# yardenas/ethz-safe-learning

Hardware: AMD Instinct MI355X
Metric: planning steps/sec (CEM-MPC, N=2000 K=5 H=30) (higher is better)
Workload: dtype f32

## Files before the change

ethz_safe_learning_amd/_capi.py:

```python
from __future__ import annotations

import ctypes as C
import os

CEM_ABI_VERSION = 4
CEM_MAX_ACT = 32
CEM_MAX_COST_KINDS = 4
CEM_COMM_ID_BYTES = 128
CEM_MAX_BATCH = 256
CEM_TRAIN_MAX_BATCH = 4096
CEM_INIT_COLD, CEM_INIT_EXPLICIT, CEM_INIT_SHIFT = 0, 1, 2
CEM_VARIANT_CEM, CEM_VARIANT_SAFE, CEM_VARIANT_COST = 0, 1, 2
CEM_PARTICLES_MEAN, CEM_PARTICLES_LOWER_TAIL = 0, 1
CEM_CONSTRAINT_BETA, CEM_CONSTRAINT_BUDGET = 0, 1
CEM_REFIT_UNIFORM, CEM_REFIT_SOFTMAX = 0, 1
CEM_NOISE_WHITE, CEM_NOISE_MIXED = 0, 1
CEM_FORWARD_SPLIT, CEM_FORWARD_ALL = 0, 1

_HERE = os.path.dirname(os.path.abspath(__file__))
LIB_PATH = os.environ.get('CEM_MPC_LIB') or os.path.join(_HERE, 'lib', 'libcem_mpc_gfx950.so')

EXPORTED_SYMBOLS = [
    'cem_abi_version', 'cem_status_string', 'cem_last_hip_error', 'cem_weight_blob_floats',
    'cem_packed_weight_floats', 'cem_workspace_bytes', 'cem_pack_weights_host', 'cem_plan_tiles_host', 'cem_plan_segments_host', 'cem_rollout_residency',
    'cem_planner_create', 'cem_planner_destroy', 'cem_planner_layout', 'cem_planner_set_weights', 'cem_planner_set_weights_dev',
    'cem_planner_set_normaliser', 'cem_planner_plan', 'cem_plan_begin', 'cem_plan_rollout', 'cem_plan_select',
    'cem_plan_end', 'cem_comm_unique_id', 'cem_planner_comm_init', 'cem_planner_comm_destroy', 'cem_planner_comm_ranks', 'cem_plan_exchange', 'cem_planner_graph_status', 'cem_planner_launches_per_iteration', 'cem_planner_rollout_path', 'cem_unfold_sequences', 'cem_compute_objective', 'cem_scorer_reward', 'cem_scorer_cost', 'cem_fill_noise', 'cem_philox_words', 'cem_planner_set_timing', 'cem_planner_last_timing', 'cem_planner_last_timing_detail', 'cem_planner_select_mode', 'cem_planner_inject_fault',
    'cem_batch_workspace_bytes', 'cem_batch_planner_create', 'cem_planner_plan_batch', 'cem_planner_batch_capacity',
    'cem_planner_set_warm_start', 'cem_planner_set_initial_distribution', 'cem_planner_set_init_mode', 'cem_planner_reset_carry',
    'cem_planner_get_carry', 'cem_planner_set_carry_slots', 'cem_planner_set_particle_objective', 'cem_planner_get_particle_objective',
    'cem_planner_set_constraint', 'cem_planner_get_constraint', 'cem_planner_set_cost_budget', 'cem_planner_constraint_costs',
    'cem_planner_set_refit', 'cem_planner_get_refit', 'cem_planner_refit_stats',
    'cem_planner_set_action_noise', 'cem_planner_get_action_noise', 'cem_planner_action_noise_dev',
    'cem_trainer_workspace_bytes', 'cem_trainer_blob_floats', 'cem_trainer_create', 'cem_trainer_destroy', 'cem_trainer_set_state',
    'cem_trainer_get_state', 'cem_trainer_weights_dev', 'cem_trainer_step', 'cem_trainer_steps', 'cem_trainer_eval', 'cem_trainer_forward',
]


class CemScorer(C.Structure):
    _fields_ = [
        ('goal_mode', C.c_int32), ('goal_lo', C.c_int32), ('goal_hi', C.c_int32),
        ('lidar_max_dist', C.c_float), ('goal_size', C.c_float), ('goal_reached_dist', C.c_float), ('reward_distance', C.c_float),
        ('reward_goal', C.c_float), ('reward_clip', C.c_float),
        ('constrain_indicator', C.c_int32), ('n_cost_kinds', C.c_int32),
        ('cost_lo', C.c_int32 * CEM_MAX_COST_KINDS), ('cost_hi', C.c_int32 * CEM_MAX_COST_KINDS),
        ('cost_size', C.c_float * CEM_MAX_COST_KINDS),
    ]


class CemConfig(C.Structure):
    _fields_ = [
        ('abi_version', C.c_int32), ('obs_dim', C.c_int32), ('act_dim', C.c_int32),
        ('units', C.c_int32), ('n_layers', C.c_int32), ('activation', C.c_int32), ('ensemble_size', C.c_int32),
        ('particles', C.c_int32), ('n_samples', C.c_int32), ('horizon', C.c_int32),
        ('n_elite', C.c_int32), ('iterations', C.c_int32),
        ('smoothing', C.c_float), ('one_minus_smoothing', C.c_float), ('stddev_threshold', C.c_float), ('noise_stddev', C.c_float),
        ('variant', C.c_int32), ('posterior_mean_threashold', C.c_float),
        ('sampling_propagation', C.c_int32), ('scale_features', C.c_int32),
        ('act_lb', C.c_float * CEM_MAX_ACT), ('act_ub', C.c_float * CEM_MAX_ACT),
        ('act_mu0', C.c_float * CEM_MAX_ACT), ('act_sigma0', C.c_float * CEM_MAX_ACT),
# ... 43 lines not shown
    vp, fp, i32p = C.c_void_p, C.POINTER(C.c_float), C.POINTER(C.c_int32)
    cfgp = C.POINTER(CemConfig)
    lib.cem_abi_version.restype = C.c_int
    lib.cem_status_string.restype = C.c_char_p
    lib.cem_status_string.argtypes = [C.c_int]
    lib.cem_last_hip_error.restype = C.c_int
    for f in ('cem_weight_blob_floats', 'cem_packed_weight_floats', 'cem_workspace_bytes'):
        getattr(lib, f).restype = C.c_size_t
        getattr(lib, f).argtypes = [cfgp]
    lib.cem_pack_weights_host.argtypes = [cfgp, vp, vp]
    lib.cem_plan_tiles_host.argtypes = [cfgp, i32p, i32p, vp, C.c_int32]
    lib.cem_plan_segments_host.argtypes = [cfgp, i32p, i32p]
    lib.cem_rollout_residency.argtypes = [C.c_int32, C.c_int32, i32p, i32p]
    lib.cem_planner_create.argtypes = [cfgp, vp, C.c_size_t, vp, C.POINTER(vp)]
    lib.cem_planner_destroy.argtypes = [vp]
    lib.cem_planner_layout.argtypes = [vp, C.POINTER(CemLayout)]
    lib.cem_planner_set_weights.argtypes = [vp, vp, C.c_size_t]
    lib.cem_planner_set_weights_dev.argtypes = [vp, vp, C.c_size_t]
    lib.cem_planner_set_normaliser.argtypes = [vp, vp, vp]
    lib.cem_planner_plan.argtypes = [vp, vp, C.c_uint64, C.c_uint64, vp, vp, vp, vp, fp, i32p]
    lib.cem_plan_begin.argtypes = [vp, vp, C.c_uint64, C.c_uint64, vp, vp]
    lib.cem_plan_rollout.argtypes = [vp, C.c_int32]
    lib.cem_plan_select.argtypes = [vp, C.c_int32]
    lib.cem_plan_end.argtypes = [vp, vp, vp, fp, i32p]
    lib.cem_unfold_sequences.argtypes = [vp, vp, vp, C.c_int32, C.c_int32, vp, C.c_uint64, C.c_uint64, vp, vp, vp]
    lib.cem_comm_unique_id.argtypes = [vp]
    lib.cem_planner_comm_init.argtypes = [vp, vp, C.c_int32, C.c_int32]
    lib.cem_planner_comm_destroy.argtypes = [vp]
    lib.cem_plan_exchange.argtypes = [vp]
    lib.cem_planner_graph_status.argtypes = [vp, i32p]
    lib.cem_planner_comm_ranks.argtypes = [vp, i32p]
    lib.cem_planner_launches_per_iteration.argtypes = [vp, i32p]
    lib.cem_planner_rollout_path.argtypes = [vp, i32p]
    lib.cem_compute_objective.argtypes = [vp, vp, C.c_int32, C.c_int32, vp]
    lib.cem_scorer_reward.argtypes = [vp, vp, vp, C.c_int32, vp, vp]
    lib.cem_scorer_cost.argtypes = [vp, vp, C.c_int32, vp]
    lib.cem_fill_noise.argtypes = [vp, C.c_uint64, C.c_uint64, vp, vp, vp]
    lib.cem_philox_words.argtypes = [vp, C.c_uint64, C.c_uint64] + [C.c_uint32] * 6 + [vp]
    lib.cem_planner_select_mode.argtypes = [vp, i32p]
    lib.cem_planner_inject_fault.argtypes = [vp, C.c_int32]
    lib.cem_planner_set_timing.argtypes = [vp, C.c_int32]
    lib.cem_planner_last_timing.argtypes = [vp, fp, i32p, fp]
    lib.cem_planner_last_timing_detail.argtypes = [vp, fp, fp]
    lib.cem_batch_workspace_bytes.restype = C.c_size_t
    lib.cem_batch_workspace_bytes.argtypes = [cfgp, C.c_int32]
    lib.cem_batch_planner_create.argtypes = [cfgp, C.c_int32, vp, C.c_size_t, vp, C.POINTER(vp)]
    lib.cem_planner_plan_batch.argtypes = [vp, C.c_int32, vp, C.c_uint64, vp, vp, vp, vp, vp, vp, vp]
    lib.cem_planner_batch_capacity.argtypes = [vp, i32p]
    lib.cem_planner_set_warm_start.argtypes = [vp, C.POINTER(CemWarmStart)]
    lib.cem_planner_set_initial_distribution.argtypes = [vp, C.c_int32, vp, vp]
    lib.cem_planner_set_init_mode.argtypes = [vp, C.c_int32, C.c_int32]
    lib.cem_planner_reset_carry.argtypes = [vp, C.c_int32]
    lib.cem_planner_get_carry.argtypes = [vp, C.c_int32, vp, vp, i32p]
    lib.cem_planner_set_carry_slots.argtypes = [vp, C.c_int32, vp]
    lib.cem_planner_set_particle_objective.argtypes = [vp, C.c_int32, C.c_int32]
    lib.cem_planner_get_particle_objective.argtypes = [vp, i32p, i32p]
    lib.cem_planner_set_constraint.argtypes = [vp, C.c_int32, C.c_int32]
    lib.cem_planner_get_constraint.argtypes = [vp, i32p, i32p]
    lib.cem_planner_set_cost_budget.argtypes = [vp, vp, C.c_int32]
    lib.cem_planner_constraint_costs.argtypes = [vp, C.c_int32, vp, C.c_int32]
    lib.cem_planner_set_refit.argtypes = [vp, C.c_int32, C.c_float]
    lib.cem_planner_get_refit.argtypes = [vp, i32p, fp]
    lib.cem_planner_refit_stats.argtypes = [vp, C.c_int32, vp, C.c_int32]
    lib.cem_planner_set_action_noise.argtypes = [vp, C.c_int32, vp]
    lib.cem_planner_get_action_noise.argtypes = [vp, i32p, vp]
    lib.cem_planner_action_noise_dev.argtypes = [vp, C.POINTER(vp), C.POINTER(C.c_size_t)]
# ... 28 lines not shown
```

ethz_safe_learning_amd/csrc/cem_capi.hip:

```cpp
#include "cem_device.h"
#include "cem_rollout_lean.h"
#include "cem_score.h"
#include "cem_refit_weighted.h"
#include "cem_noise_mix.h"
#include "cem_train.h"
#include "cem_train_tile.h"
#include "cem_forward.h"
#include "cem_rollout_split.h"
#include "cem_rollout_wide.h"
#include "cem_pack.h"
#include "../../include/cem_mpc.h"

#include <dlfcn.h>
#include <link.h>

#include <algorithm>
#include <atomic>
#include <chrono>
#include <cmath>
#include <cstdio>
#include <cstdlib>
#include <cstring>
#include <limits>
#include <mutex>
// ... 1968 lines not shown
    int n = 0;
    NCCLCHK(r->CommCount(h->comm, &n));
    *n_ranks_out = n;
    return CEM_OK;
}

int cem_planner_comm_destroy(cem_planner_t *h)
{
    if (!h) return CEM_ERR_INVALID_ARG;
    if (h->in_plan) return CEM_ERR_STATE;
    if (h->comm) {
        HIPCHK(hipStreamSynchronize(h->stream));
        if (Rccl *r = rccl()) r->CommDestroy(h->comm);
        h->comm = nullptr;
        drop_graph(h);
    }
    return CEM_OK;
}

int cem_planner_graph_status(const cem_planner_t *h, int32_t *status_out)
{
    if (!h || !status_out) return CEM_ERR_INVALID_ARG;
    *status_out = h->graph_ready ? 1 : (h->graph_failed ? 2 : 0);
    return CEM_OK;
}

int cem_planner_rollout_path(const cem_planner_t *h, int32_t *path_out)
{
    if (!h || !path_out) return CEM_ERR_INVALID_ARG;
    *path_out = (h->lean_rollout && h->noise_kind != CEM_NOISE_MIXED) ? 1 : 0;
    return CEM_OK;
}

int cem_planner_launches_per_iteration(const cem_planner_t *h, int32_t *launches_out)
{
    if (!h || !launches_out) return CEM_ERR_INVALID_ARG;
    const int mode = select_mode_now(h);
    *launches_out = 1 + (h->sample_in_rollout ? 0 : 1) + (folds_reduce(h) ? 0 : 1) + (mode == 2 ? 8 : (mode == 3 ? 2 : 1)) +
                    (h->refit_kind == CEM_REFIT_SOFTMAX ? 1 : 0);
    return CEM_OK;
}

int cem_plan_exchange(cem_planner_t *h)
{
    if (!h) return CEM_ERR_INVALID_ARG;
    if (!h->in_plan || !h->comm) return CEM_ERR_STATE;
    return enqueue_exchange(h);
}

static int ensure_scratch(cem_planner *h, size_t bytes)
{
    if (bytes <= h->scratch_bytes) return CEM_OK;
    if (h->scratch) { HIPCHK(hipStreamSynchronize(h->stream)); HIPCHK(hipFree(h->scratch)); h->scratch = nullptr; h->scratch_bytes = 0; }
    const size_t want = align256(bytes + bytes / 2);
    HIPCHK(hipMalloc((void **)&h->scratch, want));
    h->scratch_bytes = want;
    return CEM_OK;
}

static int upload_key(cem_planner *h, uint64_t seed, uint64_t call)
{
    CtrlBlock *c = h->h_ctrl;
    c->seed_lo = (uint32_t)seed; c->seed_hi = (uint32_t)(seed >> 32); c->call_lo = (uint32_t)call; c->call_hi = (uint32_t)(call >> 32);
    HIPCHK(hipMemcpyAsync(h->ws + h->lay.ctrl, c, 16, hipMemcpyHostToDevice, h->stream));
    return CEM_OK;
}
// ... 449 lines not shown
```

ethz_safe_learning_amd/csrc/cem_rollout_lean.h:

```cpp
#pragma once
#include "cem_device.h"

#define CEM_LEAN_ACT_LDS_BYTES(H_, AZ_) (((size_t)(H_) + 1) * (AZ_) * (32 + 17 * 16))
#define CEM_LEAN_LDS_BYTES(H_, AZ_) (CEM_ROLLOUT_LDS_BYTES(1) + CEM_LEAN_ACT_LDS_BYTES(H_, AZ_))
#define CEM_LEAN_ACT_LDS_MAX 16384

__attribute__((weak)) hipError_t launch_rollout_lean(const RolloutParams &p, int grid, hipStream_t st, bool seg);
```

ethz_safe_learning_amd/csrc/cem_rollout_lean.hip:

```cpp
#define CEM_DEVICE_PRIMITIVES_ONLY
#include "cem_rollout_lean.h"

namespace {

template <int V> struct LeanConst { static constexpr int value = V; };

template <int KF, int NOWN, bool L0IN>
__device__ __forceinline__ void cem_lean_stage(f4 (&acc0)[1], f4 (&acc1)[1], f4 (&hB)[CEM_NG][1], WRing &wq, const char *const *rb, const int xoff)
{
    static_assert(KF % 4 == 0, "stage lengths must keep the ring phase");
#pragma unroll
    for (int P = 0; P < KF; ++P) {
        wq.slot[(P + 3) & 3] = wq.ld(wq.pos);
        wq.pos = (wq.pos + 1 == wq.n) ? 0 : wq.pos + 1;
        __builtin_amdgcn_sched_barrier(0);
        if (P == 1) {
            __syncthreads();
#pragma unroll
            for (int Q = NOWN; Q < KF; ++Q) hB[Q][0] = *reinterpret_cast<const f4 *>(rb[Q - NOWN] + xoff + (Q - NOWN) * 1024);
        }
        const AGroup g = wq.slot[P & 3];
        const int Pb = (!L0IN && P < 2) ? (P ^ 1) : P;
#pragma unroll
        for (int r = 0; r < 4; ++r) {
            acc0[0] = CEM_MFMA(g.a[r], hB[P][0][r], acc0[0]);
            acc1[0] = CEM_MFMA(g.b[r], hB[Pb][0][r], acc1[0]);
        }
    }
}

template <bool SEG>
__device__ __forceinline__ void cem_lean_tile(const RolloutParams &p, char *smem, const int tile_idx, const int t_begin, const int t_end)
{
    constexpr int RC = 1, NFW = 1;
    const int tid = (int)((threadIdx.x + 64u * (unsigned)((tile_idx + (tile_idx >> 8)) & 3)) & 255u);
    const int w = __builtin_amdgcn_readfirstlane(tid >> 6);
    const int lane = tid & 63;
    const int j = lane & 15, q = lane >> 4;
    const TileDesc td = p.tiles[tile_idx];
    const bool resumed = SEG && t_begin > 0;
    const int wbk = 0;
    const __amdgpu_buffer_rsrc_t seg_rs = __builtin_amdgcn_make_buffer_rsrc(
        SEG ? const_cast<f4 *>(p.seg_state + (size_t)(tile_idx - p.n_pinned) * (2 * 256 + 64)) : const_cast<f4 *>(p.wpack), 0, (2 * 256 + 64) * 16, 0x00020000);
    const int O = p.O, A = p.A, H = p.H, AZ = (A + 3) >> 2;
    constexpr int XB = CEM_NG * 1024;
    float *part = reinterpret_cast<float *>(smem + 2 * XB);
    const CtrlBlock *const ctrl = p.ctrl;
    const PhiloxKey key = cem_key(ctrl);
    const float rscale = p.sampling ? CEM_BM_RSCALE : 0.0f;

    const int member_u = __builtin_amdgcn_readfirstlane(td.member);
    WRing wq;
    wq.init(p.wpack + (size_t)member_u * p.member_stride_f4 + p.wave_off_f4[w], lane, (int)p.wave_groups[w]);

    const __amdgpu_buffer_rsrc_t et_rs = __builtin_amdgcn_make_buffer_rsrc(
        const_cast<float *>(p.etab + (size_t)member_u * (CEM_ET_ROWS + p.L) * CEM_U), 0, (CEM_ET_ROWS + p.L) * CEM_U * 4, 0x00020000);
    const int tab_v = 64 * w + 16 * q;
    const int bias_v = 128 * w + 16 * q;
    const char *tabl = smem + 2 * XB + CEM_PART_FLOATS * 4;
    const char *actl = tabl + CEM_TAB_LDS_BYTES;
    {
        const int ht = (int)threadIdx.x;
        *reinterpret_cast<f4 *>(const_cast<char *>(tabl) + ht * 16) = cem_ld_tab(et_rs, (ht & 31) * 16, (ht >> 5) * 512);
        const int HA = H * A;
// ... 21 lines not shown
                float v = 0.f;
                if (f < O) v = td.s0_base < 0 ? ctrl->state[f] : p.s0[(size_t)(td.s0_base + slot0) * O + f];
                s[0][0][r] = v;
            }
        }
    }

    const int zq = 4 * w + q - (O >> 2);
    const bool actlane = zq >= 0 && zq < AZ;
    const bool wact = 4 * w + 3 >= (O >> 2) && 4 * w < (O >> 2) + AZ;
    const int zc = actlane ? zq : 0;
    const uint32_t pc0 = (uint32_t)((actlane ? td.act_base : td.noise_row_base) + slot0);
    const uint32_t pc2 = actlane ? ((uint32_t)zc | (CEM_STREAM_ACT << 16)) : ((uint32_t)(4 * w + q) | (CEM_STREAM_MODEL << 16));
    const uint32_t pc1 = ((uint32_t)p.it << 16) + (actlane ? 1u : 0u);
    const float prs = actlane ? CEM_BM_RSCALE : rscale;
    const char *const actl_v = actl + zc * 32;
#define CEM_LEAN_ACTION(DST, E_, T_) do { \
        const char *m_ = actl_v + (T_) * AZ * 32, *b_ = actl_v + H * AZ * 32; \
        const f4 sg_ = *reinterpret_cast<const f4 *>(m_), mu_ = *reinterpret_cast<const f4 *>(m_ + 16); \
        const f4 lb_ = *reinterpret_cast<const f4 *>(b_), ub_ = *reinterpret_cast<const f4 *>(b_ + 16); \
        f4 v_ = (E_) * sg_; v_ = v_ + mu_; \
        _Pragma("unroll") for (int r = 0; r < 4; ++r) DST[r] = fminf(fmaxf(v_[r], lb_[r]), ub_[r]); } while (0)
    const bool act_keep = actlane && j < td.cnt && td.row_base < p.Nloc;
    char *const stage = const_cast<char *>(actl) + (H + 1) * AZ * 32;
    char *const stage_v = stage + ((act_keep ? j : 16) * (H + 1) * AZ + zc) * 16;
#define CEM_LEAN_KEEP(V_, T_) do { *reinterpret_cast<f4 *>(stage_v + (T_) * AZ * 16) = (V_); } while (0)

    float d_prev = 0.f, c_prev = 0.f, cum = 0.f;
    bool done = false;
    const int nk = 1 + p.sc.n_cost;
    const float csz[4] = {p.sc.cost_size[0], p.sc.cost_size[1], p.sc.cost_size[2], p.sc.cost_size[3]};
    const float ind_cap = p.sc.indicator ? 1.0f : __builtin_inff(), clipv = p.sc.reward_clip > 0.f ? p.sc.reward_clip : __builtin_inff();
    const __amdgpu_buffer_rsrc_t cost_rs = __builtin_amdgcn_make_buffer_rsrc(p.costs, 0, p.costs ? (uint32_t)(H * p.Bloc) : 0u, 0x00020000);

    f4 hB[CEM_NG][RC];
    if (resumed) {
        const f4 x = cem_ld_coherent(seg_rs, (256 + tid) * 16);
        hB[0][0] = x;
        *reinterpret_cast<f4 *>(smem + (w * 64 + lane) * 16) = x;
        if (w == wbk) {
            const f4 b = cem_ld_coherent(seg_rs, (2 * 256 + lane) * 16);
            d_prev = b[0]; c_prev = b[1]; cum = b[2]; done = b[3] != 0.f;
        }
    } else {
        float pm[2][RC];
        pm[0][0] = __builtin_inff(); pm[1][0] = __builtin_inff();
        const int tv = tab_v;
        const f4 mn4 = CEM_TAB(tabl, CEM_ET_NMIN, tv), rd4 = CEM_TAB(tabl, CEM_ET_RDELTA, tv);
        const f4 isact4 = CEM_TAB(tabl, CEM_ET_ACT, tv);
        const f4 sel0 = CEM_TAB(tabl, CEM_ET_SEL0, tv), sel1 = CEM_TAB(tabl, CEM_ET_SEL1, tv);
        const f4 e0 = cem_normal4(pc0, 0u, (uint32_t)p.it, (uint32_t)zc, CEM_STREAM_ACT, key);
        const f4 sn = s[0][0];
        f4 xin = sn;
        if (wact) {
            f4 act4; CEM_LEAN_ACTION(act4, e0, 0);
            CEM_LEAN_KEEP(act4, 0);
            xin = __builtin_elementwise_fma(isact4, act4, sn);
        }
        cem_scorer_terms(sn, p.sc.D, sel0, sel1, pm[0][0], pm[1][0]);
        const f4 x = cem_sub4(xin, mn4) * rd4;
        *reinterpret_cast<f4 *>(smem + (w * 64 + lane) * 16) = x;
        hB[0][0] = x;
        CEM_RARE_KINDS_AND_STORE(RC, NFW, p, part, w, q, j, nk, s, pm, tab_v, CEM_SEL0_LDS, tabl);
    }
    f4 nb0 = cem_ld_tab(et_rs, bias_v, CEM_ET_ROWS * 512);
    f4 nb1 = cem_ld_tab(et_rs, bias_v + 64, CEM_ET_ROWS * 512);

    const char *rbh[6], *rb0[3];
#pragma unroll
    for (int k = 0; k < 6; ++k) rbh[k] = smem + lane * 16 + (k < 2 * w ? 0 : 2048);
#pragma unroll
    for (int k = 0; k < 3; ++k) rb0[k] = smem + lane * 16 + (k < w ? 0 : 1024);
    char *const pubh = smem + (2 * w * 64 + lane) * 16, *const pub0 = smem + (w * 64 + lane) * 16;
    const bool prio_rot = !(SEG && tile_idx >= p.n_pinned);
    const int prio_r0 = (tile_idx >> 8) % 3;
    auto step = [&](auto XW0, const int t, const bool first) __attribute__((always_inline)) {
        int xw = decltype(XW0)::value;
        if (prio_rot) {
            const int lvl = (t + prio_r0) % 3;
            if (lvl == 0) __builtin_amdgcn_s_setprio(0); else if (lvl == 1) __builtin_amdgcn_s_setprio(1); else __builtin_amdgcn_s_setprio(2);
        }
#define CEM_RELU_PUBLISH() do { \
            f4 h0 = acc0[0], h1 = acc1[0]; \
            _Pragma("unroll") for (int r = 0; r < 4; ++r) { h0[r] = fmaxf(h0[r], 0.f); h1[r] = fmaxf(h1[r], 0.f); } \
            *reinterpret_cast<f4 *>(pubh + xw) = h0; \
            *reinterpret_cast<f4 *>(pubh + xw + 1024) = h1; \
            hB[0][0] = h0; hB[1][0] = h1; \
            xw ^= XB; } while (0)
#define CEM_NEXT_BIAS(LN) do { \
            nb0 = cem_ld_tab(et_rs, bias_v, (CEM_ET_ROWS + (LN)) * 512); \
            nb1 = cem_ld_tab(et_rs, bias_v + 64, (CEM_ET_ROWS + (LN)) * 512); } while (0)
        {
            f4 acc0[RC], acc1[RC];
            acc0[0] = nb0; acc1[0] = nb1;
            CEM_NEXT_BIAS(1);
            cem_lean_stage<4, 1, true>(acc0, acc1, hB, wq, rb0, xw ^ XB);
            if (!(resumed && first)) CEM_BOOKKEEP(p, td, part, w, wbk, lane, nk, csz, ind_cap, clipv, cost_rs, d_prev, c_prev, cum, done, t - 1);
            CEM_RELU_PUBLISH();
        }
#pragma unroll
        for (int l = 1; l < 4; ++l) {
            f4 acc0[RC], acc1[RC];
            acc0[0] = nb0; acc1[0] = nb1;
            CEM_NEXT_BIAS(l + 1 < 4 ? l + 1 : 0);
            cem_lean_stage<CEM_NG, 2, false>(acc0, acc1, hB, wq, rbh, xw ^ XB);
            CEM_RELU_PUBLISH();
        }
#undef CEM_RELU_PUBLISH
#undef CEM_NEXT_BIAS

        float pm[2][RC];
        pm[0][0] = __builtin_inff(); pm[1][0] = __builtin_inff();
        const int tn = (t + 1 < H) ? t + 1 : H - 1;
        {
            const int Fo = w;
            const int tv = tab_v;
            f4 accm[RC], accv[RC];
            accm[0] = CEM_TAB(tabl, CEM_ET_BMU, tv); accv[0] = CEM_TAB(tabl, CEM_ET_BVAR, tv);
            if (Fo < p.KB_obs) cem_lean_stage<CEM_NG, 2, false>(accm, accv, hB, wq, rbh, xw ^ XB);
            else __syncthreads();
            const f4 e4 = cem_normal4(pc0, pc1 + (uint32_t)t, 0u, pc2, 0u, key, prs);
            const f4 mn4 = CEM_TAB(tabl, CEM_ET_NMIN, tv), rd4 = CEM_TAB(tabl, CEM_ET_RDELTA, tv);
            const f4 om4 = CEM_TAB(tabl, CEM_ET_OBS, tv), isact4 = CEM_TAB(tabl, CEM_ET_ACT, tv);
            const f4 sel0 = CEM_TAB(tabl, CEM_ET_SEL0, tv), sel1 = CEM_TAB(tabl, CEM_ET_SEL1, tv);

            const f4 mu = accm[0];
            const f4 var = cem_softplus4(accv[0]) + 1e-4f;
            f4 sd;
#pragma unroll
            for (int r = 0; r < 4; ++r) sd[r] = __builtin_amdgcn_sqrtf(var[r]);
            const f4 d = mu + sd * e4;
            const f4 sn = s[0][0] + d * om4;
            s[0][0] = sn;
            cem_scorer_terms(sn, p.sc.D, sel0, sel1, pm[0][0], pm[1][0]);
            f4 xin = sn;
            if (wact) {
                f4 act4; CEM_LEAN_ACTION(act4, e4, tn);
                CEM_LEAN_KEEP(act4, t + 1);
                xin = __builtin_elementwise_fma(isact4, act4, sn);
            }
            const f4 x = cem_sub4(xin, mn4) * rd4;
            *reinterpret_cast<f4 *>(pub0 + xw) = x;
            hB[0][0] = x;
        }
        CEM_RARE_KINDS_AND_STORE(RC, NFW, p, part, w, q, j, nk, s, pm, tab_v, CEM_SEL0_LDS, tabl);
    };
    for (int t = t_begin; t < t_end; t += 2) {
        step(LeanConst<XB>{}, t, t == t_begin);
        if (t + 1 >= t_end) break;
        step(LeanConst<0>{}, t + 1, false);
    }
#undef CEM_LEAN_ACTION
#undef CEM_LEAN_KEEP
    __syncthreads();
    CEM_BOOKKEEP(p, td, part, w, wbk, lane, nk, csz, ind_cap, clipv, cost_rs, d_prev, c_prev, cum, done, t_end - 1);
    if (td.row_base < p.Nloc) {
        const int tlo = resumed ? t_begin + 1 : 0, thi = t_end < H ? t_end : H - 1;
        const int per = (thi - tlo + 1) * A;
        const float *const stagef = reinterpret_cast<const float *>(stage);
        for (int idx = (int)threadIdx.x; idx < td.cnt * per; idx += 256) {
            const int row = idx / per, rem = idx - row * per, tt = tlo + rem / A, a = rem - (rem / A) * A;
            p.actions_w[((size_t)(td.act_base + row) * H + tt) * A + a] = stagef[((row * (H + 1) + tt) * AZ) * 4 + a];
        }
    }
    if (!SEG || t_end == H) {
        if (w == wbk && lane < td.cnt) p.ret[td.row_base + lane] = cum;
    } else {
        cem_st_coherent(seg_rs, tid * 16, s[0][0]);
        cem_st_coherent(seg_rs, (256 + tid) * 16, hB[0][0]);
        if (w == wbk) cem_st_coherent(seg_rs, (2 * 256 + lane) * 16, (f4){d_prev, c_prev, cum, done ? 1.0f : 0.0f});
    }
}

}

__global__ __launch_bounds__(256) void cem_rollout_lean_kernel(const RolloutParams p)
{
    extern __shared__ __attribute__((aligned(16))) char smem[];
    if (p.check_done && p.ctrl->done) return;
    cem_lean_tile<false>(p, smem, (int)blockIdx.x, 0, p.H);
}

__global__ __launch_bounds__(256) void cem_rollout_lean_seg_kernel(const RolloutParams p)
{
    extern __shared__ __attribute__((aligned(16))) char smem[];
    __shared__ uint32_t item_s;
    if (p.check_done && p.ctrl->done) return;
    if ((int)blockIdx.x < p.n_pinned) {
        cem_lean_tile<true>(p, smem, (int)blockIdx.x, 0, p.H);
        return;
    }
    __builtin_amdgcn_s_setprio(CEM_FLOAT_PRIO);
    const uint32_t n_float = (uint32_t)(p.n_tiles - p.n_pinned);
    if (threadIdx.x == 0) {
        const uint32_t ticket = atomicAdd(p.seg_queue, 1u);
        uint32_t item = (((uint32_t)p.n_pinned + ticket) << 8);
        if (ticket >= n_float) {
            const uint32_t *slot = p.seg_flags + (ticket - n_float);
            uint32_t spins = 0, v;
            while ((v = __hip_atomic_load(slot, __ATOMIC_RELAXED, __HIP_MEMORY_SCOPE_AGENT)) == 0u && ++spins < CEM_SEG_SPIN_LIMIT)
                __builtin_amdgcn_s_sleep(16);
            item = v ? v - 1u : 0xffffffffu;
            if (!v) atomicOr(const_cast<int32_t *>(&p.ctrl->fault), 1 );
        }
        item_s = item;
    }
    __syncthreads();
    const uint32_t item = item_s;
    if (item == 0xffffffffu) return;
    const int tile = (int)(item >> 8), seg = (int)(item & 255u);
    const int t0 = seg * p.seg_len, t1 = (t0 + p.seg_len < p.H) ? t0 + p.seg_len : p.H;
    cem_lean_tile<true>(p, smem, tile, t0, t1);
    if (t1 == p.H) {
        if (threadIdx.x == 0) item_s = atomicAdd(p.seg_queue + 2, 1u);
        __syncthreads();
        if (item_s == n_float - 1u) {
            const int n_ready = (int)n_float * (p.n_seg - 1);
            for (int i = (int)threadIdx.x; i < n_ready; i += 256) __hip_atomic_store(p.seg_flags + i, 0u, __ATOMIC_RELAXED, __HIP_MEMORY_SCOPE_AGENT);
            if (threadIdx.x < 3) __hip_atomic_store(p.seg_queue + threadIdx.x, 0u, __ATOMIC_RELAXED, __HIP_MEMORY_SCOPE_AGENT);
        }
    }
    if (t1 < p.H) {
        __builtin_amdgcn_s_waitcnt(0x0F70);
        __syncthreads();
        if (threadIdx.x == 0) {
            const uint32_t pos = atomicAdd(p.seg_queue + 1, 1u);
            __hip_atomic_store(p.seg_flags + pos, (((uint32_t)tile << 8) | (uint32_t)(seg + 1)) + 1u, __ATOMIC_RELAXED, __HIP_MEMORY_SCOPE_AGENT);
        }
    }
}

hipError_t launch_rollout_lean(const RolloutParams &p, int grid, hipStream_t st, bool seg)
{
    const size_t lds = CEM_LEAN_LDS_BYTES(p.H, (p.A + 3) / 4);
    if (seg) hipLaunchKernelGGL(cem_rollout_lean_seg_kernel, dim3(grid), dim3(256), lds, st, p);
    else hipLaunchKernelGGL(cem_rollout_lean_kernel, dim3(grid), dim3(256), lds, st, p);
    return hipGetLastError();
}
```

ethz_safe_learning_amd/planner.py:

```python
from __future__ import annotations

import ctypes as C
import math
from dataclasses import dataclass, field
from typing import List, Optional, Sequence, Tuple

import numpy as np

from . import _capi


@dataclass
class ScorerConfig:
    goal_slice: Tuple[int, int]
    observe_goal_lidar: bool = True
    lidar_max_dist: float = 4.0
    goal_size: float = 0.3
    reward_distance: float = 1.0
    reward_goal: float = 1.0
    reward_clip: float = 10.0
    constrain_indicator: bool = True
    cost_kinds: List[Tuple[int, int, float]] = field(default_factory=list)


# ... 375 lines not shown
            src = dist.get_global_rank(group, 0) if group is not None else 0
            dist.broadcast_object_list(box, src=src, group=group)
            buf.raw = box[0]
        else:
            _capi.check(self.lib.cem_comm_unique_id(buf), 'cem_comm_unique_id')
        with self._torch.cuda.device(self.device):
            _capi.check(self.lib.cem_planner_comm_init(self.h, buf, c.world_size, c.rank), 'cem_planner_comm_init')
        self.has_comm = True

    def comm_ranks(self):
        n = C.c_int32()
        _capi.check(self.lib.cem_planner_comm_ranks(self.h, C.byref(n)), 'cem_planner_comm_ranks')
        return n.value

    def comm_destroy(self):
        _capi.check(self.lib.cem_planner_comm_destroy(self.h), 'cem_planner_comm_destroy')
        self.has_comm = False

    def graph_status(self):
        st = C.c_int32()
        _capi.check(self.lib.cem_planner_graph_status(self.h, C.byref(st)), 'cem_planner_graph_status')
        return ('eager', 'graph', 'graph-unsupported')[st.value]

    def launches_per_iteration(self):
        n = C.c_int32()
        _capi.check(self.lib.cem_planner_launches_per_iteration(self.h, C.byref(n)), 'cem_planner_launches_per_iteration')
        return n.value

    def rollout_path(self):
        n = C.c_int32()
        _capi.check(self.lib.cem_planner_rollout_path(self.h, C.byref(n)), 'cem_planner_rollout_path')
        return ('generic', 'lean')[n.value]

    def set_particle_objective(self, kind='mean', m=0):
        if kind not in PARTICLE_OBJECTIVES:
            raise ValueError("kind is 'mean' or 'lower_tail'")
        _capi.check(self.lib.cem_planner_set_particle_objective(self.h, PARTICLE_OBJECTIVES[kind], int(m)), 'cem_planner_set_particle_objective')

    def particle_objective(self):
        kind, m = C.c_int32(), C.c_int32()
        _capi.check(self.lib.cem_planner_get_particle_objective(self.h, C.byref(kind), C.byref(m)), 'cem_planner_get_particle_objective')
        return ('mean', 'lower_tail')[kind.value], m.value

    def set_constraint(self, kind='beta', worst_cost_particles=0):
        if kind not in CONSTRAINTS:
            raise ValueError("kind is 'beta' or 'budget'")
        _capi.check(self.lib.cem_planner_set_constraint(self.h, CONSTRAINTS[kind], int(worst_cost_particles)), 'cem_planner_set_constraint')

    def constraint(self):
        kind, m = C.c_int32(), C.c_int32()
        _capi.check(self.lib.cem_planner_get_constraint(self.h, C.byref(kind), C.byref(m)), 'cem_planner_get_constraint')
        return ('beta', 'budget')[kind.value], m.value

    def set_cost_budget(self, budget):
        b = np.ascontiguousarray(np.asarray(budget, np.float32).reshape(-1))
        self.budget_staged = None
        _capi.check(self.lib.cem_planner_set_cost_budget(self.h, _np_ptr(b), b.size), 'cem_planner_set_cost_budget')

    def constraint_costs(self, problem=0, n=None):
        out = np.zeros(self.n_local if n is None else int(n), np.float32)
        _capi.check(self.lib.cem_planner_constraint_costs(self.h, int(problem), _np_ptr(out), out.size), 'cem_planner_constraint_costs')
        return out

    def set_refit(self, kind='uniform', temperature=0.0):
        if kind not in REFITS:
            raise ValueError("kind is 'uniform' or 'softmax'")
# ... 453 lines not shown
```

include/cem_mpc.h:

```cpp
#ifndef CEM_MPC_H
#define CEM_MPC_H

#include <stddef.h>
#include <stdint.h>

#ifdef __cplusplus
extern "C" {
#endif

#define CEM_ABI_VERSION 4
#define CEM_MAX_ACT 32
#define CEM_MAX_COST_KINDS 4
#define CEM_MAX_BATCH 256

enum cem_status {
    CEM_OK = 0,
    CEM_ERR_INVALID_ARG = 1,
    CEM_ERR_UNSUPPORTED = 2,
    CEM_ERR_SPLIT = 3,
    CEM_ERR_WORKSPACE = 4,
    CEM_ERR_HIP = 5,
    CEM_ERR_NO_WEIGHTS = 6,
    CEM_ERR_STATE = 7,
    CEM_ERR_COMM = 8,
// ... 85 lines not shown
int cem_plan_segments_host(const cem_config_t *cfg, int32_t *segments_out, int32_t *steps_per_segment_out);

int cem_rollout_residency(int32_t chunks_per_tile, int32_t input_blocks_per_wave, int32_t *table_out, int32_t *runtime_out);

int cem_planner_create(const cem_config_t *cfg, void *workspace, size_t workspace_bytes, void *hip_stream, cem_planner_t **out);
int cem_planner_destroy(cem_planner_t *h);
int cem_planner_layout(const cem_planner_t *h, cem_layout_t *out);

int cem_planner_set_weights(cem_planner_t *h, const float *blob, size_t n_floats);
int cem_planner_set_normaliser(cem_planner_t *h, const float *inputs_min, const float *inputs_max );
int cem_planner_set_weights_dev(cem_planner_t *h, const float *blob_dev, size_t n_floats);

int cem_planner_plan(cem_planner_t *h, const float *state, uint64_t seed, uint64_t call,
                     const float *eps_act_dev, const float *eps_model_dev, const float *eps_out_host,
                     float *action_out, float *best_score_out, int32_t *iters_out);

int cem_plan_begin(cem_planner_t *h, const float *state, uint64_t seed, uint64_t call,
                   const float *eps_act_dev, const float *eps_model_dev);
int cem_plan_rollout(cem_planner_t *h, int32_t it);
int cem_plan_select(cem_planner_t *h, int32_t it);
int cem_plan_end(cem_planner_t *h, const float *eps_out_host, float *action_out, float *best_score_out, int32_t *iters_out);

#define CEM_COMM_ID_BYTES 128
int cem_comm_unique_id(void *id_out );
int cem_planner_comm_init(cem_planner_t *h, const void *id , int32_t n_ranks, int32_t rank);
int cem_planner_comm_destroy(cem_planner_t *h);
int cem_planner_comm_ranks(const cem_planner_t *h, int32_t *n_ranks_out);
int cem_plan_exchange(cem_planner_t *h);
int cem_planner_select_mode(const cem_planner_t *h, int32_t *mode_out);
int cem_planner_inject_fault(cem_planner_t *h, int32_t kind);
int cem_planner_graph_status(const cem_planner_t *h, int32_t *status_out);
int cem_planner_launches_per_iteration(const cem_planner_t *h, int32_t *launches_out);
int cem_planner_rollout_path(const cem_planner_t *h, int32_t *path_out);

int cem_unfold_sequences(cem_planner_t *h, const float *s0_dev, const float *actions_dev, int32_t n_rows, int32_t horizon,
                         const float *eps_model_dev, uint64_t seed, uint64_t call,
                         float *traj_out_dev, float *mu_out_dev, float *sd_out_dev);

int cem_compute_objective(cem_planner_t *h, const float *traj_dev, int32_t n_rows, int32_t horizon, float *scores_out_dev);

int cem_scorer_reward(cem_planner_t *h, const float *obs_dev, const float *next_obs_dev, int32_t n, float *reward_out_dev,
                      uint8_t *goal_achieved_out_dev);
int cem_scorer_cost(cem_planner_t *h, const float *obs_dev, int32_t n, float *cost_out_dev);

int cem_fill_noise(cem_planner_t *h, uint64_t seed, uint64_t call, float *eps_act_dev, float *eps_model_dev, float *eps_out_dev);

int cem_philox_words(cem_planner_t *h, uint64_t seed, uint64_t call, uint32_t stream, uint32_t iteration, uint32_t t, uint32_t sub,
                     uint32_t idx0, uint32_t n, uint32_t *words_out_dev);

int cem_planner_set_timing(cem_planner_t *h, int32_t enable);
int cem_planner_last_timing(cem_planner_t *h, float *rollout_ms_total, int32_t *rollout_launches, float *select_ms_total);
int cem_planner_last_timing_detail(cem_planner_t *h, float *reduce_ms_total, float *sampler_ms_total);

size_t cem_batch_workspace_bytes(const cem_config_t *cfg, int32_t max_batch);
int cem_batch_planner_create(const cem_config_t *cfg, int32_t max_batch, void *workspace, size_t workspace_bytes, void *hip_stream,
                             cem_planner_t **out);
int cem_planner_plan_batch(cem_planner_t *h, int32_t n_states, const float *states, uint64_t seed, const uint64_t *calls,
                           const float *eps_act_dev, const float *eps_model_dev, const float *eps_out_host, float *actions_out,
                           float *best_scores_out, int32_t *iters_out);
int cem_planner_batch_capacity(const cem_planner_t *h, int32_t *max_batch_out);

enum cem_init_mode { CEM_INIT_COLD = 0, CEM_INIT_EXPLICIT = 1, CEM_INIT_SHIFT = 2 };
typedef struct cem_warm_start {
    int32_t shift;
    int32_t tail;
    int32_t sigma_rule;
// ... 73 lines not shown
```

Before: 544.3.

## Defer lean rollout reward bookkeeping to a post-loop LDS settle pass

In the lean rollout kernel, per-step scorer outputs are logged into an extra LDS region instead of running the serial per-step bookkeeping inside the time loop. After the loop, a parallel settle pass computes rewards, goal-first masks via atomicMin, cost stores and the cumulative sum. This aims to take the bookkeeping latency off the critical recurrent path. In exchange it raises LDS use per workgroup, which can reduce occupancy. It also adds query APIs that report which bookkeeping form is used and the resulting residency.

```diff
diff --git a/ethz_safe_learning_amd/_capi.py b/ethz_safe_learning_amd/_capi.py
--- a/ethz_safe_learning_amd/_capi.py
+++ b/ethz_safe_learning_amd/_capi.py
@@ -25,7 +25,7 @@
     'cem_packed_weight_floats', 'cem_workspace_bytes', 'cem_pack_weights_host', 'cem_plan_tiles_host', 'cem_plan_segments_host', 'cem_rollout_residency',
     'cem_planner_create', 'cem_planner_destroy', 'cem_planner_layout', 'cem_planner_set_weights', 'cem_planner_set_weights_dev',
     'cem_planner_set_normaliser', 'cem_planner_plan', 'cem_plan_begin', 'cem_plan_rollout', 'cem_plan_select',
-    'cem_plan_end', 'cem_comm_unique_id', 'cem_planner_comm_init', 'cem_planner_comm_destroy', 'cem_planner_comm_ranks', 'cem_plan_exchange', 'cem_planner_graph_status', 'cem_planner_launches_per_iteration', 'cem_planner_rollout_path', 'cem_unfold_sequences', 'cem_compute_objective', 'cem_scorer_reward', 'cem_scorer_cost', 'cem_fill_noise', 'cem_philox_words', 'cem_planner_set_timing', 'cem_planner_last_timing', 'cem_planner_last_timing_detail', 'cem_planner_select_mode', 'cem_planner_inject_fault',
+    'cem_plan_end', 'cem_comm_unique_id', 'cem_planner_comm_init', 'cem_planner_comm_destroy', 'cem_planner_comm_ranks', 'cem_plan_exchange', 'cem_planner_graph_status', 'cem_planner_launches_per_iteration', 'cem_planner_rollout_path', 'cem_planner_lean_bookkeeping', 'cem_rollout_lean_residency', 'cem_unfold_sequences', 'cem_compute_objective', 'cem_scorer_reward', 'cem_scorer_cost', 'cem_fill_noise', 'cem_philox_words', 'cem_planner_set_timing', 'cem_planner_last_timing', 'cem_planner_last_timing_detail', 'cem_planner_select_mode', 'cem_planner_inject_fault',
     'cem_batch_workspace_bytes', 'cem_batch_planner_create', 'cem_planner_plan_batch', 'cem_planner_batch_capacity',
     'cem_planner_set_warm_start', 'cem_planner_set_initial_distribution', 'cem_planner_set_init_mode', 'cem_planner_reset_carry',
     'cem_planner_get_carry', 'cem_planner_set_carry_slots', 'cem_planner_set_particle_objective', 'cem_planner_get_particle_objective',
@@ -135,6 +135,8 @@
     lib.cem_planner_comm_ranks.argtypes = [vp, i32p]
     lib.cem_planner_launches_per_iteration.argtypes = [vp, i32p]
     lib.cem_planner_rollout_path.argtypes = [vp, i32p]
+    lib.cem_planner_lean_bookkeeping.argtypes = [vp, i32p]
+    lib.cem_rollout_lean_residency.argtypes = [C.c_int32, C.c_int32, C.c_int32, i32p]
     lib.cem_compute_objective.argtypes = [vp, vp, C.c_int32, C.c_int32, vp]
     lib.cem_scorer_reward.argtypes = [vp, vp, vp, C.c_int32, vp, vp]
     lib.cem_scorer_cost.argtypes = [vp, vp, C.c_int32, vp]
diff --git a/ethz_safe_learning_amd/csrc/cem_capi.hip b/ethz_safe_learning_amd/csrc/cem_capi.hip
--- a/ethz_safe_learning_amd/csrc/cem_capi.hip
+++ b/ethz_safe_learning_amd/csrc/cem_capi.hip
@@ -2024,6 +2024,23 @@
     return CEM_OK;
 }
 
+int cem_planner_lean_bookkeeping(const cem_planner_t *h, int32_t *form_out)
+{
+    if (!h || !form_out) return CEM_ERR_INVALID_ARG;
+    const bool lean = h->lean_rollout && h->noise_kind != CEM_NOISE_MIXED;
+    *form_out = !lean ? 0 : (CEM_LEAN_LOG_FITS(h->d.H, (h->d.A + 3) / 4, 1 + h->cfg.scorer.n_cost_kinds) ? 2 : 1);
+    return CEM_OK;
+}
+
+int cem_rollout_lean_residency(int32_t horizon, int32_t act_dim, int32_t n_cost_kinds, int32_t *runtime_out)
+{
+    if (horizon < 1 || act_dim < 1 || act_dim > CEM_MAX_ACT || n_cost_kinds < 0 || n_cost_kinds > CEM_MAX_COST_KINDS || !runtime_out) return CEM_ERR_INVALID_ARG;
+    if (CEM_LEAN_ACT_LDS_BYTES(horizon, (act_dim + 3) / 4) > CEM_LEAN_ACT_LDS_MAX) return CEM_ERR_INVALID_ARG;
+    if (query_lean_resident == nullptr) return CEM_ERR_UNSUPPORTED;
+    for (int seg = 0; seg < 2; ++seg) runtime_out[seg] = query_lean_resident(horizon, act_dim, n_cost_kinds, seg != 0);
+    return CEM_OK;
+}
+
 int cem_planner_launches_per_iteration(const cem_planner_t *h, int32_t *launches_out)
 {
     if (!h || !launches_out) return CEM_ERR_INVALID_ARG;
diff --git a/ethz_safe_learning_amd/csrc/cem_rollout_lean.h b/ethz_safe_learning_amd/csrc/cem_rollout_lean.h
--- a/ethz_safe_learning_amd/csrc/cem_rollout_lean.h
+++ b/ethz_safe_learning_amd/csrc/cem_rollout_lean.h
@@ -5,4 +5,11 @@
 #define CEM_LEAN_LDS_BYTES(H_, AZ_) (CEM_ROLLOUT_LDS_BYTES(1) + CEM_LEAN_ACT_LDS_BYTES(H_, AZ_))
 #define CEM_LEAN_ACT_LDS_MAX 16384
 
+#define CEM_LEAN_LOG_LDS_MAX 16384
+#define CEM_LEAN_WG_LDS_MAX 53248
+#define CEM_LEAN_LOG_LDS_BYTES(H_, NK_) ((size_t)(((H_) + 4) / 4) * (NK_) * 1024)
+#define CEM_LEAN_LOG_FITS(H_, AZ_, NK_) (CEM_LEAN_LOG_LDS_BYTES(H_, NK_) <= CEM_LEAN_LOG_LDS_MAX && \
+                                         CEM_LEAN_LDS_BYTES(H_, AZ_) + CEM_LEAN_LOG_LDS_BYTES(H_, NK_) <= CEM_LEAN_WG_LDS_MAX)
+
 __attribute__((weak)) hipError_t launch_rollout_lean(const RolloutParams &p, int grid, hipStream_t st, bool seg);
+__attribute__((weak)) int query_lean_resident(int H, int A, int n_cost, bool seg);
diff --git a/ethz_safe_learning_amd/csrc/cem_rollout_lean.hip b/ethz_safe_learning_amd/csrc/cem_rollout_lean.hip
--- a/ethz_safe_learning_amd/csrc/cem_rollout_lean.hip
+++ b/ethz_safe_learning_amd/csrc/cem_rollout_lean.hip
@@ -29,7 +29,68 @@
     }
 }
 
-template <bool SEG>
+#define CEM_LEAN_SLOT(LOGB_, NK_, I_) ((LOGB_) + ((I_) >> 2) * (NK_) * 256 + 16 * ((I_) & 3))
+
+#define CEM_LEAN_SCR_FIRST 0
+#define CEM_LEAN_SCR_DONE0 16
+#define CEM_LEAN_SCR_DLAST 32
+#define CEM_LEAN_SCR_CLAST 48
+#define CEM_LEAN_SCR_R 96
+#define CEM_LEAN_MIN4(SL_) fminf(fminf((SL_)[0], (SL_)[64]), fminf((SL_)[128], (SL_)[192]))
+__device__ __forceinline__ float cem_lean_cost_count(const RolloutParams &p, const float *sl, const int nk)
+{
+    float cn = 0.f;
+#pragma unroll
+    for (int k = 1; k < CEM_NKIND; ++k)
+        if (k < nk) { const float dk = CEM_LEAN_MIN4(sl + k * 256); cn = cn + ((dk <= p.sc.cost_size[k - 1]) ? 1.0f : 0.0f); }
+    return fminf(cn, p.sc.indicator ? 1.0f : __builtin_inff());
+}
+__device__ __forceinline__ void cem_lean_settle(const RolloutParams &p, const TileDesc &td, const float *logb, float *scr, const int nk, const bool resumed,
+                                                const int t_begin, const int n, const bool bkwave, const int lane, float &d_prev, float &c_prev, float &cum, bool &done)
+{
+    const float clipv = p.sc.reward_clip > 0.f ? p.sc.reward_clip : __builtin_inff();
+    uint32_t *const first = reinterpret_cast<uint32_t *>(scr) + CEM_LEAN_SCR_FIRST;
+    const uint32_t *const done0 = reinterpret_cast<const uint32_t *>(scr) + CEM_LEAN_SCR_DONE0;
+    for (int idx = (int)threadIdx.x + 16; idx < 16 * (n + 1); idx += 256) {
+        const int i = idx >> 4, row = idx & 15;
+        const float *const sl = CEM_LEAN_SLOT(logb, nk, i) + row, *const pv = CEM_LEAN_SLOT(logb, nk, i - 1) + row;
+        const float dp = (resumed && i == 1) ? pv[0] : CEM_LEAN_MIN4(pv), dn = CEM_LEAN_MIN4(sl);
+        const bool ga = dp <= p.sc.goal_thresh;
+        float r = (dp - dn) * p.sc.reward_distance + (ga ? 1.0f : 0.0f) * p.sc.reward_goal;
+        r = fminf(fmaxf(r, -clipv), clipv);
+        scr[CEM_LEAN_SCR_R + idx] = r;
+        if (ga) atomicMin(first + row, (uint32_t)i);
+        if (i == n) { scr[CEM_LEAN_SCR_DLAST + row] = dn; scr[CEM_LEAN_SCR_CLAST + row] = cem_lean_cost_count(p, sl, nk); }
+    }
+    __syncthreads();
+    const __amdgpu_buffer_rsrc_t cost_rs = __builtin_amdgcn_make_buffer_rsrc(p.costs, 0, p.costs ? (uint32_t)(p.H * p.Bloc) : 0u, 0x00020000);
+    for (int idx = (int)threadIdx.x + 16; idx < 16 * (n + 1); idx += 256) {
+        const int i = idx >> 4, row = idx & 15;
+        const bool masked = done0[row] != 0u || (p.variant == 1 ? first[row] <= (uint32_t)i : first[row] < (uint32_t)i);
+        const float nd = masked ? 0.0f : 1.0f;
+        scr[CEM_LEAN_SCR_R + idx] = scr[CEM_LEAN_SCR_R + idx] * nd;
+        if (p.variant == 1 && p.costs && row < td.cnt) {
+            const float *const pv = CEM_LEAN_SLOT(logb, nk, i - 1) + row;
+            const float cst = ((resumed && i == 1) ? pv[64] : cem_lean_cost_count(p, pv, nk)) * nd;
+            __builtin_amdgcn_raw_buffer_store_b8((uint8_t)cst, cost_rs, (t_begin + i - 1) * p.Bloc + td.row_base + row, 0, 0);
+        }
+    }
+    __syncthreads();
+    if (bkwave) {
+        const int row = lane & 15;
+        for (int i0 = 1; i0 <= n; i0 += 8) {
+            float v[8];
+#pragma unroll
+            for (int u = 0; u < 8; ++u) v[u] = scr[CEM_LEAN_SCR_R + 16 * (i0 + u <= n ? i0 + u : n) + row];
+#pragma unroll
+            for (int u = 0; u < 8; ++u) if (i0 + u <= n) cum = cum + v[u];
+        }
+        done = done || first[row] <= (uint32_t)n;
+        d_prev = scr[CEM_LEAN_SCR_DLAST + row]; c_prev = scr[CEM_LEAN_SCR_CLAST + row];
+    }
+}
+
+template <bool SEG, bool LOG>
 __device__ __forceinline__ void cem_lean_tile(const RolloutParams &p, char *smem, const int tile_idx, const int t_begin, const int t_end)
 {
     constexpr int RC = 1, NFW = 1;
@@ -117,6 +178,10 @@
     const float csz[4] = {p.sc.cost_size[0], p.sc.cost_size[1], p.sc.cost_size[2], p.sc.cost_size[3]};
     const float ind_cap = p.sc.indicator ? 1.0f : __builtin_inff(), clipv = p.sc.reward_clip > 0.f ? p.sc.reward_clip : __builtin_inff();
     const __amdgpu_buffer_rsrc_t cost_rs = __builtin_amdgcn_make_buffer_rsrc(p.costs, 0, p.costs ? (uint32_t)(H * p.Bloc) : 0u, 0x00020000);
+    float *const logb = reinterpret_cast<float *>(smem + CEM_LEAN_LDS_BYTES(H, AZ));
+    float *plog = LOG ? logb : part;
+    int pslot = 0;
+#define CEM_LEAN_LOG_NEXT() do { if (LOG) { plog += (pslot & 3) == 3 ? nk * 256 - 48 : 16; ++pslot; } } while (0)
 
     f4 hB[CEM_NG][RC];
     if (resumed) {
@@ -126,6 +191,10 @@
         if (w == wbk) {
             const f4 b = cem_ld_coherent(seg_rs, (2 * 256 + lane) * 16);
             d_prev = b[0]; c_prev = b[1]; cum = b[2]; done = b[3] != 0.f;
+            if (LOG && lane < 16) {
+                logb[lane] = b[0]; logb[64 + lane] = b[1];
+                reinterpret_cast<uint32_t *>(part)[CEM_LEAN_SCR_DONE0 + lane] = done ? 1u : 0u;
+            }
         }
     } else {
         float pm[2][RC];
@@ -146,7 +215,12 @@
         const f4 x = cem_sub4(xin, mn4) * rd4;
         *reinterpret_cast<f4 *>(smem + (w * 64 + lane) * 16) = x;
         hB[0][0] = x;
-        CEM_RARE_KINDS_AND_STORE(RC, NFW, p, part, w, q, j, nk, s, pm, tab_v, CEM_SEL0_LDS, tabl);
+        CEM_RARE_KINDS_AND_STORE(RC, NFW, p, plog, w, q, j, nk, s, pm, tab_v, CEM_SEL0_LDS, tabl);
+    }
+    CEM_LEAN_LOG_NEXT();
+    if (LOG && w == wbk && lane < 16) {
+        reinterpret_cast<uint32_t *>(part)[CEM_LEAN_SCR_FIRST + lane] = 0x7fffffffu;
+        if (!resumed) reinterpret_cast<uint32_t *>(part)[CEM_LEAN_SCR_DONE0 + lane] = 0u;
     }
     f4 nb0 = cem_ld_tab(et_rs, bias_v, CEM_ET_ROWS * 512);
     f4 nb1 = cem_ld_tab(et_rs, bias_v + 64, CEM_ET_ROWS * 512);
@@ -180,7 +254,9 @@
             acc0[0] = nb0; acc1[0] = nb1;
             CEM_NEXT_BIAS(1);
             cem_lean_stage<4, 1, true>(acc0, acc1, hB, wq, rb0, xw ^ XB);
-            if (!(resumed && first)) CEM_BOOKKEEP(p, td, part, w, wbk, lane, nk, csz, ind_cap, clipv, cost_rs, d_prev, c_prev, cum, done, t - 1);
+#ifndef CEM_DBG_NOBOOKKEEP
+            if (!LOG && !(resumed && first)) CEM_BOOKKEEP(p, td, part, w, wbk, lane, nk, csz, ind_cap, clipv, cost_rs, d_prev, c_prev, cum, done, t - 1);
+#endif
             CEM_RELU_PUBLISH();
         }
 #pragma unroll
@@ -218,17 +294,17 @@
             const f4 sn = s[0][0] + d * om4;
             s[0][0] = sn;
             cem_scorer_terms(sn, p.sc.D, sel0, sel1, pm[0][0], pm[1][0]);
-            f4 xin = sn;
+            f4 x;
             if (wact) {
                 f4 act4; CEM_LEAN_ACTION(act4, e4, tn);
                 CEM_LEAN_KEEP(act4, t + 1);
-                xin = __builtin_elementwise_fma(isact4, act4, sn);
-            }
-            const f4 x = cem_sub4(xin, mn4) * rd4;
+                x = cem_sub4(__builtin_elementwise_fma(isact4, act4, sn), mn4) * rd4;
+            } else x = cem_sub4(sn, mn4) * rd4;
             *reinterpret_cast<f4 *>(pub0 + xw) = x;
             hB[0][0] = x;
         }
-        CEM_RARE_KINDS_AND_STORE(RC, NFW, p, part, w, q, j, nk, s, pm, tab_v, CEM_SEL0_LDS, tabl);
+        CEM_RARE_KINDS_AND_STORE(RC, NFW, p, plog, w, q, j, nk, s, pm, tab_v, CEM_SEL0_LDS, tabl);
+        CEM_LEAN_LOG_NEXT();
     };
     for (int t = t_begin; t < t_end; t += 2) {
         step(LeanConst<XB>{}, t, t == t_begin);
@@ -237,8 +313,10 @@
     }
 #undef CEM_LEAN_ACTION
 #undef CEM_LEAN_KEEP
+#undef CEM_LEAN_LOG_NEXT
     __syncthreads();
-    CEM_BOOKKEEP(p, td, part, w, wbk, lane, nk, csz, ind_cap, clipv, cost_rs, d_prev, c_prev, cum, done, t_end - 1);
+    if (LOG) cem_lean_settle(p, td, logb, part, nk, resumed, t_begin, t_end - t_begin, w == wbk, lane, d_prev, c_prev, cum, done);
+    else CEM_BOOKKEEP(p, td, part, w, wbk, lane, nk, csz, ind_cap, clipv, cost_rs, d_prev, c_prev, cum, done, t_end - 1);
     if (td.row_base < p.Nloc) {
         const int tlo = resumed ? t_begin + 1 : 0, thi = t_end < H ? t_end : H - 1;
         const int per = (thi - tlo + 1) * A;
@@ -257,13 +335,28 @@
     }
 }
 
+__device__ __forceinline__ bool cem_lean_logs(const RolloutParams &p)
+{
+#ifdef CEM_DBG_NOBOOKKEEP
+    return false;
+#else
+    return CEM_LEAN_LOG_FITS(p.H, (p.A + 3) >> 2, 1 + p.sc.n_cost);
+#endif
+}
+template <bool SEG>
+__device__ __forceinline__ void cem_lean_tile_any(const RolloutParams &p, char *smem, const int tile_idx, const int t_begin, const int t_end)
+{
+    if (cem_lean_logs(p)) cem_lean_tile<SEG, true>(p, smem, tile_idx, t_begin, t_end);
+    else cem_lean_tile<SEG, false>(p, smem, tile_idx, t_begin, t_end);
+}
+
 }
 
 __global__ __launch_bounds__(256) void cem_rollout_lean_kernel(const RolloutParams p)
 {
     extern __shared__ __attribute__((aligned(16))) char smem[];
     if (p.check_done && p.ctrl->done) return;
-    cem_lean_tile<false>(p, smem, (int)blockIdx.x, 0, p.H);
+    cem_lean_tile_any<false>(p, smem, (int)blockIdx.x, 0, p.H);
 }
 
 __global__ __launch_bounds__(256) void cem_rollout_lean_seg_kernel(const RolloutParams p)
@@ -272,7 +365,7 @@
     __shared__ uint32_t item_s;
     if (p.check_done && p.ctrl->done) return;
     if ((int)blockIdx.x < p.n_pinned) {
-        cem_lean_tile<true>(p, smem, (int)blockIdx.x, 0, p.H);
+        cem_lean_tile_any<true>(p, smem, (int)blockIdx.x, 0, p.H);
         return;
     }
     __builtin_amdgcn_s_setprio(CEM_FLOAT_PRIO);
@@ -295,7 +388,7 @@
     if (item == 0xffffffffu) return;
     const int tile = (int)(item >> 8), seg = (int)(item & 255u);
     const int t0 = seg * p.seg_len, t1 = (t0 + p.seg_len < p.H) ? t0 + p.seg_len : p.H;
-    cem_lean_tile<true>(p, smem, tile, t0, t1);
+    cem_lean_tile_any<true>(p, smem, tile, t0, t1);
     if (t1 == p.H) {
         if (threadIdx.x == 0) item_s = atomicAdd(p.seg_queue + 2, 1u);
         __syncthreads();
@@ -315,10 +408,33 @@
     }
 }
 
+static bool lean_logs(const int H, const int A, const int n_cost)
+{
+#ifdef CEM_DBG_NOBOOKKEEP
+    return false;
+#else
+    return CEM_LEAN_LOG_FITS(H, (A + 3) / 4, 1 + n_cost);
+#endif
+}
+static size_t lean_lds(const int H, const int A, const int n_cost)
+{
+    return CEM_LEAN_LDS_BYTES(H, (A + 3) / 4) + (lean_logs(H, A, n_cost) ? CEM_LEAN_LOG_LDS_BYTES(H, 1 + n_cost) : 0);
+}
+
 hipError_t launch_rollout_lean(const RolloutParams &p, int grid, hipStream_t st, bool seg)
 {
-    const size_t lds = CEM_LEAN_LDS_BYTES(p.H, (p.A + 3) / 4);
+    const size_t lds = lean_lds(p.H, p.A, p.sc.n_cost);
     if (seg) hipLaunchKernelGGL(cem_rollout_lean_seg_kernel, dim3(grid), dim3(256), lds, st, p);
     else hipLaunchKernelGGL(cem_rollout_lean_kernel, dim3(grid), dim3(256), lds, st, p);
     return hipGetLastError();
 }
+
+int query_lean_resident(int H, int A, int n_cost, bool seg)
+{
+    int n = 0;
+    const size_t lds = lean_lds(H, A, n_cost);
+    const hipError_t e = seg ? hipOccupancyMaxActiveBlocksPerMultiprocessor(&n, cem_rollout_lean_seg_kernel, 256, lds)
+                             : hipOccupancyMaxActiveBlocksPerMultiprocessor(&n, cem_rollout_lean_kernel, 256, lds);
+    if (e != hipSuccess || n < 1) { (void)hipGetLastError(); return 0; }
+    return n;
+}
diff --git a/ethz_safe_learning_amd/planner.py b/ethz_safe_learning_amd/planner.py
--- a/ethz_safe_learning_amd/planner.py
+++ b/ethz_safe_learning_amd/planner.py
@@ -431,6 +431,11 @@
         _capi.check(self.lib.cem_planner_rollout_path(self.h, C.byref(n)), 'cem_planner_rollout_path')
         return ('generic', 'lean')[n.value]
 
+    def lean_bookkeeping(self):
+        n = C.c_int32()
+        _capi.check(self.lib.cem_planner_lean_bookkeeping(self.h, C.byref(n)), 'cem_planner_lean_bookkeeping')
+        return (None, 'step', 'settle')[n.value]
+
     def set_particle_objective(self, kind='mean', m=0):
         if kind not in PARTICLE_OBJECTIVES:
             raise ValueError("kind is 'mean' or 'lower_tail'")
diff --git a/include/cem_mpc.h b/include/cem_mpc.h
--- a/include/cem_mpc.h
+++ b/include/cem_mpc.h
@@ -141,6 +141,8 @@
 int cem_planner_graph_status(const cem_planner_t *h, int32_t *status_out);
 int cem_planner_launches_per_iteration(const cem_planner_t *h, int32_t *launches_out);
 int cem_planner_rollout_path(const cem_planner_t *h, int32_t *path_out);
+int cem_planner_lean_bookkeeping(const cem_planner_t *h, int32_t *form_out);
+int cem_rollout_lean_residency(int32_t horizon, int32_t act_dim, int32_t n_cost_kinds, int32_t *runtime_out);
 
 int cem_unfold_sequences(cem_planner_t *h, const float *s0_dev, const float *actions_dev, int32_t n_rows, int32_t horizon,
                          const float *eps_model_dev, uint64_t seed, uint64_t call,
```

New measurement: 547.2, median of 6. Within noise of the previous version (+0.5%).
